# Lingeng56/conformer-pytorch-lightning

Hardware: AMD Instinct MI355X
Metric: encoder frames/sec (80-d fbank, T=1000), whole job (higher is better)
Workload: dtype bf16

## Files before the change

conformer-pytorch-lightning_amd/cfm/__init__.py:

```python
import ctypes
import os
import threading

import torch

_HERE = os.path.dirname(os.path.abspath(__file__))
LIB_PATH = os.path.join(os.path.dirname(_HERE), "libconformer_gfx950.so")

F32, BF16, F16 = 0, 1, 2
ACT_NONE, ACT_SILU, ACT_RELU, ACT_GLU, ACT_DSILU, ACT_DRELU = 0, 1, 2, 3, 4, 5
TILE_AUTO_TRAIN = -1

_DT = {torch.float32: F32, torch.bfloat16: BF16, torch.float16: F16}
_TORCH_DT = {F32: torch.float32, BF16: torch.bfloat16, F16: torch.float16}

c_p = ctypes.c_void_p
c_i64 = ctypes.c_int64
c_i32 = ctypes.c_int32
c_f = ctypes.c_float


class GemmDesc(ctypes.Structure):
    _fields_ = [("A", c_p), ("W", c_p), ("W_lo", c_p), ("bias", c_p), ("residual", c_p), ("row_mask", c_p), ("C", c_p),
                ("lda", c_i64), ("ldc", c_i64), ("ldr", c_i64),
# ... 134 lines not shown
    _fields_ = [("lat", Lattice), ("logits", c_p), ("ld", c_i64), ("logits_dtype", c_i32), ("V", c_i32), ("blank", c_i32), ("ld_targets", c_i32),
                ("targets", c_p), ("lse", c_p), ("lp_blank", c_p), ("lp_label", c_p), ("alpha", c_p), ("beta", c_p), ("shift", c_p),
                ("nll", c_p), ("nll_shifted", c_p), ("ll_alpha", c_p),
                ("grad", c_p), ("ld_grad", c_i64), ("grad_dtype", c_i32), ("grad_cols", c_i32), ("gscale", ctypes.c_float),
                ("gscale_stride", c_i32), ("gscale_dev", c_p), ("clamp", ctypes.c_float)]


class LnBwdDesc(ctypes.Structure):
    _fields_ = [("x", c_p), ("dy", c_p), ("gamma", c_p), ("row_mask", c_p), ("dres", c_p), ("dx", c_p), ("dgamma", c_p), ("dbeta", c_p), ("ws", c_p),
                ("dx2", c_p), ("M", c_i64), ("D", c_i32), ("dy_dtype", c_i32), ("dx2_dtype", c_i32), ("accumulate", c_i32),
                ("eps", ctypes.c_float), ("alpha2", ctypes.c_float), ("p1", ctypes.c_float), ("p2", ctypes.c_float),
                ("seed1", ctypes.c_uint32), ("seed2", ctypes.c_uint32), ("dx2_row_mask", c_p),
                ("chain_x", c_p), ("chain_gamma", c_p), ("chain_dgamma", c_p), ("chain_dbeta", c_p)]


class GreedyDesc(ctypes.Structure):
    _fields_ = [("embed", c_p), ("lstm_w", c_p * 4), ("lstm_b", c_p * 4), ("proj_w", c_p), ("proj_b", c_p), ("pf_w", c_p), ("pf_b", c_p), ("out_w", c_p),
                ("out_b", c_p), ("enc_proj", c_p), ("token", c_p), ("t", c_p), ("count", c_p), ("frame_count", c_p), ("hyps", c_p), ("lens", c_p),
                ("h", c_p), ("c", c_p), ("h_new", c_p), ("c_new", c_p), ("pred", c_p), ("act", c_p), ("pmax", c_p), ("pidx", c_p), ("done", c_p),
                ("n_done", c_p), ("hyp_cap", c_i64), ("hyp_ld", c_i64), ("B", c_i32), ("T", c_i32), ("L", c_i32), ("E", c_i32), ("H", c_i32),
                ("P", c_i32), ("J", c_i32), ("Vp", c_i32), ("blank", c_i32), ("n_steps", c_i32)]


class GreedyChunkDesc(ctypes.Structure):
    _fields_ = ([("embed", c_p), ("lstm_w", c_p * 4), ("lstm_b", c_p * 4)] +
                [(n, c_p) for n in ("proj_w", "proj_b", "pf_w", "pf_b", "out_w", "out_b", "ef_w", "ef_b", "enc", "enc_proj", "token", "t", "count", "frame_count",
                                    "hyps", "lens", "h", "c", "h_new", "c_new", "pred", "pp", "act", "pmax", "pidx", "rows", "row_off", "row_cnt", "n_rows",
                                    "steps", "overflow", "done", "n_done")] +
                [("hyp_cap", c_i64), ("hyp_ld", c_i64)] +
                [(n, c_i32) for n in ("B", "chunk", "L", "E", "H", "P", "J", "D", "Vp", "blank", "n_steps", "carry")])


class FbankDesc(ctypes.Structure):
    _fields_ = ([(n, c_p) for n in ("samples", "lengths", "feats_length", "carry_in", "carry_out", "fresh_in", "pos_in", "fresh_out", "pos_out", "twiddle", "window",
                                    "mel_w", "mel_start", "mel_len", "mel_off", "out")] + [("ld", c_i64)] +
                [(n, c_i32) for n in ("B", "n_cols", "rows", "F", "win", "shift", "padded", "mel_nnz", "samples_i16", "carry_n", "hop")] +
                [("dither", c_f), ("seed", ctypes.c_uint32)])


class FfnSplitDesc(ctypes.Structure):
    _fields_ = [("x", c_p), ("psum", c_p), ("psum_b2", c_p), ("psum_splits", c_i32), ("psum_alpha", c_f), ("ln1_g", c_p), ("ln1_b", c_p), ("ln2_g", c_p),
                ("ln2_b", c_p), ("rows_out", c_p), ("rows2_out", c_p), ("ln_g", c_p), ("ln_b", c_p), ("w1", c_p), ("b1", c_p), ("N1", c_i32), ("act", c_i32),
                ("w2", c_p), ("psum_out", c_p), ("out16", c_p), ("ldo", c_i64), ("M", c_i32), ("D", c_i32), ("mode", c_i32), ("w_dtype", c_i32), ("eps", c_f),
                ("kv_ring", c_p), ("ring_offsets", c_p), ("ring_T", c_i32), ("ring_H", c_i32), ("ring_Tq", c_i32)]


class LayerScratch(ctypes.Structure):
    _fields_ = [(n, c_p) for n in ("xn", "hid", "qkv", "pos", "ctx", "glu", "dw")] + [("psum", c_p), ("psum_splits", c_i32)]


class LayerIO(ctypes.Structure):
    _fields_ = [("B", c_i32), ("T", c_i32), ("D", c_i32), ("H", c_i32), ("FF", c_i32), ("ktaps", c_i32),
                ("act_dtype", c_i32), ("w_dtype", c_i32),
                ("attn_mask", c_p), ("am_sb", c_i64), ("am_sq", c_i64),
                ("pad_valid", c_p), ("pos_embed", c_p), ("pos_rows", c_i32),
                ("pos_proj", c_p), ("pos_proj_ld", c_i64),
                ("attn_cache", c_p), ("cache_T", c_i32), ("new_cache", c_p), ("after_g", c_p), ("after_b", c_p), ("after_out", c_p),
                ("kv_ring", c_p), ("stream_offset", c_p), ("ring_T", c_i32), ("causal_conv", c_i32), ("conv_cache", c_p), ("pos_shared", c_i32),
                ("next_w", c_p), ("next_x_out", c_p), ("macaron_done", c_i32)]


ROUTES = ("GENERAL", "FUSED_FFN", "CHAIN", "CHAIN_NEXT", "CHAIN_NEXT_CIN", "FFSPLIT", "PAIR")

_lib = None
_lock = threading.Lock()


def lib():
    global _lib
    if _lib is not None:
        return _lib
    with _lock:
        if _lib is not None:
            return _lib
        if not os.path.exists(LIB_PATH):
            raise RuntimeError(
                "libconformer_gfx950.so not found at %s -- build it with `python -c 'import __graft_entry__ as g; g.build()'` "
                "or `make -C conformer-pytorch-lightning_amd/csrc`. There is no CPU fallback." % LIB_PATH)
        L = ctypes.CDLL(LIB_PATH)
        L.cfm_version.restype = ctypes.c_int
        L.cfm_last_error.restype = ctypes.c_char_p
        L.cfm_device_ok.restype = ctypes.c_int
        L.cfm_gemm.argtypes = [ctypes.POINTER(GemmDesc), c_p]
        L.cfm_attention.argtypes = [ctypes.POINTER(AttnDesc), c_p]
        L.cfm_ffn_fused.argtypes = [ctypes.POINTER(FfnDesc), c_p]
        L.cfm_rowchain.argtypes = [ctypes.POINTER(RowChainDesc), c_p]
        L.cfm_rowchain_supported.argtypes = [c_i32, c_i32]
        L.cfm_rowchain_pair_supported.argtypes = [c_i32, c_i32]
        L.cfm_layernorm.argtypes = [c_p, c_p, c_p, c_p, c_i32, c_p, c_p, c_p, c_i32, c_p, ctypes.c_float, c_i64, c_i32, c_p]
        L.cfm_kv_cache_pack.argtypes = [c_p, c_i32, c_p, c_p, c_i32, c_i64, c_i64, c_i64, c_i64, c_p, c_i32, c_i32, c_i32, c_i32, c_p]
        L.cfm_dwconv_bn_silu.argtypes = [c_p, c_i32, c_p, c_p, c_p, c_p, c_p, c_i32, c_i32, c_i32, c_i32, c_i32, c_p]
        L.cfm_conv1_relu.argtypes = [c_p, c_p, c_p, c_p, c_i32, c_i32, c_i32, c_i32, c_i32, c_p, c_p, c_p]
        L.cfm_conv1_relu_mma.argtypes = [c_p, c_p, c_p, c_p, c_i32, c_i32, c_i32, c_i32, c_i32, c_p, c_p, c_p]
        L.cfm_conv12_supported.argtypes = [c_i32, c_i32]
        L.cfm_pack_matrices.argtypes = [c_p, c_i32, c_i64, c_i32, c_i32, c_p]
        L.cfm_pack_vectors.argtypes = [c_p, c_p, c_p, c_i64, c_p]
        L.cfm_greedy_step.argtypes = [ctypes.POINTER(GreedyDesc), c_p]
        L.cfm_greedy_chunk_begin.argtypes = [ctypes.POINTER(GreedyChunkDesc), c_p]
        L.cfm_greedy_chunk_step.argtypes = [ctypes.POINTER(GreedyChunkDesc), c_p]
        L.cfm_fbank.argtypes = [ctypes.POINTER(FbankDesc), c_p]
        L.cfm_fbank_stream.argtypes = [ctypes.POINTER(FbankDesc), c_p]
        L.cfm_ffn_split.argtypes = [ctypes.POINTER(FfnSplitDesc), c_p]
        L.cfm_ffn_split_supported.argtypes = [c_i32, c_i32]
        L.cfm_attention_bwd_force_general.argtypes = [c_i32]
        L.cfm_attention_bwd_force_general.restype = None
        L.cfm_set_cin_merge.argtypes = [c_i32]
        L.cfm_set_cin_merge.restype = c_i32
        L.cfm_set_conv12_tile.argtypes = [c_i32]
        L.cfm_set_conv12_tile.restype = c_i32
        L.cfm_conv12_plan.argtypes = [c_i64, c_i32, c_i32, ctypes.POINTER(c_i32), ctypes.POINTER(c_i32)]
        L.cfm_dwconv_bn_train_bwd_acc.argtypes = [c_p, c_i32, c_p, c_p, c_p, c_i32, c_p, c_p, c_i32, c_p, c_p, c_p, c_p, c_p, c_p, c_i32, c_i32, c_i32, c_i32, c_i32, c_p]
        L.cfm_layernorm_bwd_fused.argtypes = [ctypes.POINTER(LnBwdDesc), c_p]
        L.cfm_conv12_relu.argtypes = [c_p, c_p, c_p, c_p, c_p, c_p, c_i32, c_i32, c_i32, c_i32, c_i32, c_p, c_p, c_p]
        L.cfm_valid_mask.argtypes = [c_p, c_i32, c_p, c_i32, c_i32, c_i32, c_i32, c_p]
        L.cfm_chunk_mask.argtypes = [c_p, c_i32, c_i32, c_i32, c_p]
        L.cfm_attn_mask.argtypes = [c_p, c_p, c_p, c_i32, c_i32, c_p]
        L.cfm_cast.argtypes = [c_p, c_i32, c_p, c_i32, c_i64, c_p]
        L.cfm_add_rows.argtypes = [c_p, c_p, c_i64, c_i32, c_i32, c_p]
        L.cfm_encoder_layer_forward.argtypes = [ctypes.POINTER(LayerWeights), ctypes.POINTER(LayerScratch),
                                                ctypes.POINTER(LayerIO), c_p, c_p, c_i32, c_p, c_p, c_p]
        L.cfm_encoder_layer_route.argtypes = [ctypes.POINTER(LayerWeights), ctypes.POINTER(LayerScratch), ctypes.POINTER(LayerIO), c_p, c_p]
        L.cfm_encoder_layer_route.restype = c_i32
        L.cfm_ffsplit_max_rows.restype = c_i32
        L.cfm_ctc_nll.argtypes = [c_p, c_i64, c_i32, c_i32, c_i32, c_p, c_p, c_i32, c_p, c_p, c_p, c_p]
        L.cfm_joint_act.argtypes = [c_p, c_i64, c_p, c_i64, c_p, c_i32, c_i32, c_i32, c_i32, c_i32, c_p]
        L.cfm_joint_act_bwd.argtypes = [c_p, c_i64, c_p, c_i64, c_p, c_p, c_p, c_p, c_i32, c_i32, c_i32, c_i32, c_p]
        L.cfm_joint_act_bwd_ws.argtypes = [c_i32, c_i32, c_i32, c_i32]
        L.cfm_rnnt_nll.argtypes = [ctypes.POINTER(RnntDesc), c_p]
        L.cfm_rnnt_grad.argtypes = [ctypes.POINTER(RnntDesc), c_p]
        L.cfm_rnnt_packed_nll.argtypes = [ctypes.POINTER(RnntPackedDesc), c_p]
        L.cfm_rnnt_packed_grad.argtypes = [ctypes.POINTER(RnntPackedDesc), c_p]
        L.cfm_joint_act_packed.argtypes = [c_p, c_i64, c_p, c_i64, c_p, c_i32, ctypes.POINTER(Lattice), c_i32, c_p]
        L.cfm_joint_act_packed_bwd.argtypes = [c_p, c_i64, c_p, c_i64, c_p, c_p, c_p, c_p, ctypes.POINTER(Lattice), c_i32, c_p]
        c_f = ctypes.c_float
        L.cfm_gemm_tn.argtypes = [ctypes.POINTER(GemmTnDesc), c_p]
        L.cfm_gemm_tn_group.argtypes = [ctypes.POINTER(GemmTnDesc), c_i32, c_p]
        L.cfm_attention_bwd.argtypes = [ctypes.POINTER(AttnBwdDesc), c_p]
        L.cfm_layernorm_bwd_ws.argtypes = [c_i64, c_i32]
        L.cfm_layernorm_bwd.argtypes = [c_p, c_p, c_i32, c_p, c_p, c_p, c_p, c_p, c_p, c_p, c_f, c_i64, c_i32, c_p]
        L.cfm_glu_bwd.argtypes = [c_p, c_i32, c_p, c_i32, c_p, c_i32, c_i64, c_i32, c_p]
        L.cfm_dwconv_bn_ws.argtypes = [c_i32, c_i32, c_i32]
        L.cfm_dwconv_bn_train.argtypes = [c_p, c_i32, c_p, c_p, c_p, c_p, c_p, c_p, c_f, c_f, c_p, c_p, c_p, c_i32, c_p, c_i32, c_i32, c_i32, c_i32, c_p]
        L.cfm_dwconv_bn_train_bwd.argtypes = [c_p, c_i32, c_p, c_p, c_p, c_i32, c_p, c_p, c_i32, c_p, c_p, c_p, c_p, c_p, c_p, c_i32, c_i32, c_i32, c_i32, c_p]
        L.cfm_col2im_relu_bwd.argtypes = [c_p, c_i32, c_p, c_i32, c_p, c_i32, c_i32, c_i32, c_i32, c_i32, c_p]
        L.cfm_conv1_wgrad_ws.argtypes = [c_i32, c_i32, c_i32]
        L.cfm_conv1_wgrad.argtypes = [c_p, c_i32, c_p, c_p, c_p, c_p, c_p, c_p, c_i32, c_i32, c_i32, c_i32, c_p]
        L.cfm_ctc_nll_train_groups.argtypes = [ctypes.POINTER(CtcGroup), c_i32, c_i32, c_p]
        L.cfm_ctc_grad.argtypes = [c_p, c_i64, c_i32, c_i32, c_i32, c_p, c_p, c_i32, c_p, c_p, c_p, c_p, c_p, c_p, c_f, c_p, c_p, c_p]
        L.cfm_adam_step.argtypes = [c_p, c_p, c_p, c_p, c_i64, c_f, c_f, c_f, c_f, c_f, c_i64, c_p, c_p]
        L.cfm_sumsq.argtypes = [c_p, c_i64, c_p, c_i32, c_p, c_p]
        L.cfm_adam_clip_step.argtypes = [c_p, c_p, c_p, c_p, c_i64, c_f, c_f, c_f, c_f, c_f, c_i64, c_p, c_f, c_f, c_i32, c_p, c_p]
        L.cfm_dropout_rows.argtypes = [c_p, c_i32, c_p, c_i32, c_p, c_f, c_f, ctypes.c_uint32, c_f, ctypes.c_uint32, c_i64, c_i32, c_p]
        L.cfm_dropout_mask.argtypes = [c_p, c_i64, c_f, ctypes.c_uint32, c_p]
        L.cfm_encoder_train_forward.argtypes = [c_i32, ctypes.POINTER(LayerTrainWeights), ctypes.POINTER(LayerTrainIO), ctypes.POINTER(LayerTrainSaved),
                                                ctypes.POINTER(LayerTrainScratch), ctypes.POINTER(c_p), c_p]
        L.cfm_encoder_train_backward.argtypes = [c_i32, ctypes.POINTER(LayerTrainWeights), ctypes.POINTER(LayerTrainIO), ctypes.POINTER(LayerTrainSaved),
                                                 ctypes.POINTER(LayerTrainScratch), ctypes.POINTER(LayerTrainGrads), ctypes.POINTER(c_p), c_p, c_p, c_p,
                                                 LAYER_DONE_FN, c_p, ctypes.POINTER(c_p), c_p]
        L.cfm_stream_prep.argtypes = [c_p, c_i32, c_i32, c_i32, c_i32, c_p, c_i32, c_i32, c_p, c_p, c_p, c_p]
        L.cfm_kv_ring_write.argtypes = [c_p, c_p, c_i32, c_i64, c_i64, c_i64, c_i64, c_p, c_p, c_i32, c_i32, c_i32, c_i32, c_i32, c_p]
        L.cfm_stream_advance.argtypes = [c_p, c_p, c_i32, c_i32, c_p]
        L.cfm_dwconv_causal_bn_silu.argtypes = [c_p, c_i32, c_p, c_p, c_p, c_p, c_p, c_p, c_i32, c_i32, c_i32, c_i32, c_i32, c_p]
        L.cfm_conv_cache_update.argtypes = [c_p, c_i32, c_p, c_i32, c_i32, c_i32, c_i32, c_p]
        for name in ("cfm_layernorm_bwd_ws", "cfm_dwconv_bn_ws", "cfm_conv1_wgrad_ws", "cfm_joint_act_bwd_ws"):
            getattr(L, name).restype = c_i64
        L.cfm_prof_enable.argtypes = [c_i32]
        L.cfm_prof_enable.restype = None
        L.cfm_prof_reset.restype = None
        L.cfm_prof_collect.restype = ctypes.c_int
        L.cfm_prof_entry.argtypes = [c_i32, ctypes.c_char_p, c_i32, ctypes.POINTER(c_i64), ctypes.POINTER(ctypes.c_double),
                                     ctypes.POINTER(ctypes.c_double), ctypes.POINTER(ctypes.c_double)]
        for name in ("cfm_gemm", "cfm_ffn_fused", "cfm_rowchain", "cfm_rowchain_supported", "cfm_attention", "cfm_layernorm", "cfm_kv_cache_pack", "cfm_dwconv_bn_silu", "cfm_conv1_relu", "cfm_conv1_relu_mma", "cfm_conv12_relu", "cfm_conv12_supported",
                     "cfm_valid_mask", "cfm_chunk_mask", "cfm_attn_mask", "cfm_cast", "cfm_add_rows",
                     "cfm_encoder_layer_forward", "cfm_ctc_nll", "cfm_joint_act", "cfm_joint_act_bwd", "cfm_rnnt_nll", "cfm_rnnt_grad", "cfm_prof_entry", "cfm_gemm_tn", "cfm_gemm_tn_group", "cfm_attention_bwd",
                     "cfm_layernorm_bwd", "cfm_glu_bwd", "cfm_dwconv_bn_train", "cfm_dwconv_bn_train_bwd", "cfm_col2im_relu_bwd", "cfm_conv1_wgrad",
                     "cfm_ctc_nll_train_groups", "cfm_ctc_grad", "cfm_adam_step", "cfm_adam_clip_step", "cfm_sumsq", "cfm_dropout_rows", "cfm_dropout_mask", "cfm_pack_matrices", "cfm_pack_vectors", "cfm_greedy_step", "cfm_greedy_chunk_begin", "cfm_greedy_chunk_step", "cfm_fbank", "cfm_fbank_stream", "cfm_ffn_split", "cfm_ffn_split_supported", "cfm_layernorm_bwd_fused", "cfm_dwconv_bn_train_bwd_acc",
                     "cfm_encoder_train_forward", "cfm_encoder_train_backward", "cfm_stream_prep", "cfm_kv_ring_write", "cfm_stream_advance", "cfm_dwconv_causal_bn_silu", "cfm_conv_cache_update"):
            getattr(L, name).restype = ctypes.c_int
        _lib = L
    return _lib


def check(rc, what):
    if rc != 0:
        raise RuntimeError("%s failed (status %d): %s" % (what, rc, lib().cfm_last_error().decode(errors="replace")))


def dt_code(t):
    try:
        return _DT[t.dtype if isinstance(t, torch.Tensor) else t]
    except KeyError:
        raise TypeError("cfm: unsupported dtype %s (float32, bfloat16, float16 only)" % (t.dtype if isinstance(t, torch.Tensor) else t))


def torch_dtype(code):
    return _TORCH_DT[code]


def require_hip(*tensors):
    for t in tensors:
        if t is None:
            continue
        if not t.is_cuda:
            raise RuntimeError("cfm: tensor on %s -- this framework runs on MI355X (HIP) only; there is no CPU path" % t.device)


def ptr(t):
    return None if t is None else t.data_ptr()


def stream():
    return torch.cuda.current_stream().cuda_stream


class Precision:

    def __init__(self, name):
        if name not in ("bf16", "fp16", "fp32"):
            raise ValueError("precision must be bf16, fp16 or fp32, got %r" % (name,))
        self.name = name
        self.split = name == "fp32"
        self.w_code = F16 if name == "fp16" else BF16
        self.act_code = F32 if self.split else self.w_code
        self.w_dtype = torch_dtype(self.w_code)
        self.act_dtype = torch_dtype(self.act_code)

    def __repr__(self):
        return "Precision(%s)" % self.name


_precision = Precision(os.environ.get("CFM_PRECISION", "bf16"))


def set_precision(name):
    global _precision
    _precision = name if isinstance(name, Precision) else Precision(name)
    return _precision


def get_precision():
    return _precision


def resolve_precision(module=None):
    p = getattr(module, "precision", None) if module is not None else None
    if p is None:
        return _precision
    return p if isinstance(p, Precision) else Precision(p)


_warned = set()


def check_mode(module, what):
    if module.training:
# ... 11 lines not shown
```

conformer-pytorch-lightning_amd/cfm/ops.py:

```python
import ctypes

import torch

import cfm as _c

__all__ = ["fbank", "fbank_stream", "stream_prep", "stream_advance", "dwconv_causal_bn_silu", "conv_cache_update", "dropout_rows", "dropout_mask", "set_deterministic", "gemm_tn", "gemm_tn_group", "layernorm_bwd", "glu_bwd", "dwconv_bn_train", "dwconv_bn_train_bwd", "col2im_relu_bwd", "conv1_wgrad", "attention_bwd",
           "ctc_nll_train_groups", "ctc_grad", "rnnt_nll", "rnnt_grad", "joint_act_bwd", "rnnt_nll_packed", "joint_act_packed", "joint_act_packed_bwd", "ffn_split", "adam_step", "adam_clip_step", "sumsq", "scratch_stats",
           "gemm", "ffn_fused", "ffn_fused_supported", "rowchain", "rowchain_supported", "rowchain_pair_supported", "layernorm", "attention", "kv_cache_pack", "dwconv_bn_silu", "conv1_relu", "conv1_relu_mma_supported", "conv12_relu", "conv12_supported", "ctc_nll", "joint_act", "valid_mask", "chunk_mask",
           "attn_mask_combine", "cast", "add_rows", "scratch", "prof_enable", "prof_reset", "prof_table", "as_u8_mask"]


def _rows2d(t, name):
    if t.dim() != 2 or t.stride(1) != 1:
        raise ValueError("cfm.%s: expected a 2-D tensor with unit inner stride, got shape %s strides %s" % (name, tuple(t.shape), t.stride()))
    return t


_arena = {}
_retired = []


def scratch(tag, numel, dtype, device):
    device = torch.device(device)
    key = (tag, dtype, device, torch.cuda.current_stream(device).cuda_stream)
    buf = _arena.get(key)
    if buf is None or buf.numel() < numel:
        want = max(int(numel), 1) if buf is None else max(int(numel), buf.numel() * 3 // 2)
        if buf is not None:
            _retired.append(buf)
        buf = torch.empty(want, dtype=dtype, device=device)
        _arena[key] = buf
    return buf[:numel]


def scratch_stats():
    held = sum(b.numel() * b.element_size() for b in list(_arena.values()) + _retired)
    return len(_arena), len(_retired), held


def gemm(a, w, bias=None, w_lo=None, out=None, out_dtype=None, act=_c.ACT_NONE, residual=None, alpha=1.0, row_mask=None,
         mask_mode=0, conv=None, tile=0, n_out=None, pre_out=None, aux=None, drop=None, drop2=None):
    _c.require_hip(a, w, bias, w_lo, out, residual, row_mask)
    w = _rows2d(w, "gemm(w)")
    N, K = w.shape
    d = _c.GemmDesc()
    if conv is None:
        a = _rows2d(a, "gemm(a)")
        M = a.shape[0]
        if a.shape[1] != K:
            raise ValueError("cfm.gemm: a is %s but w is %s" % (tuple(a.shape), tuple(w.shape)))
        d.lda = a.stride(0)
    else:
        C, T1, F1, T2, F2, M = conv
        if not a.is_contiguous():
            raise ValueError("cfm.gemm(conv): image must be contiguous channels-last [B,T1,F1,C]")
        d.conv_C, d.conv_T1, d.conv_F1, d.conv_T2, d.conv_F2 = C, T1, F1, T2, F2
        d.lda = 0
    cols = N // 2 if act == _c.ACT_GLU else N
    if out is None:
        odt = out_dtype if out_dtype is not None else (residual.dtype if residual is not None else torch.float32)
        out = torch.empty((M, cols), dtype=odt, device=a.device)
    else:
        out = _rows2d(out, "gemm(out)")
        if out.shape[0] != M or out.shape[1] != cols:
            raise ValueError("cfm.gemm: out is %s, expected (%d,%d)" % (tuple(out.shape), M, cols))
    if residual is not None:
        residual = _rows2d(residual, "gemm(residual)")
        if residual.dtype != torch.float32 or out.dtype != torch.float32 or tuple(residual.shape) != (M, cols):
            raise ValueError("cfm.gemm: residual accumulate needs f32 residual/out of shape (%d,%d)" % (M, cols))
        d.ldr = residual.stride(0)
    if bias is not None and (bias.dtype != torch.float32 or bias.numel() != N or not bias.is_contiguous()):
        raise ValueError("cfm.gemm: bias must be contiguous f32 [N]")
    if row_mask is not None and (row_mask.dtype != torch.uint8 or row_mask.numel() != M or not row_mask.is_contiguous()):
        raise ValueError("cfm.gemm: row_mask must be contiguous uint8 [M]")
    if w_lo is not None and (w_lo.shape != w.shape or w_lo.dtype != w.dtype or not w_lo.is_contiguous()):
        raise ValueError("cfm.gemm: w_lo must match w")
    if pre_out is not None:
        _c.require_hip(pre_out)
        pre_out = _rows2d(pre_out, "gemm(pre_out)")
        if tuple(pre_out.shape) != (M, N):
            raise ValueError("cfm.gemm: pre_out is %s, expected (%d,%d)" % (tuple(pre_out.shape), M, N))
        d.C_pre, d.ld_pre, d.pre_dtype = _c.ptr(pre_out), pre_out.stride(0), _c.dt_code(pre_out)
    if aux is not None:
        _c.require_hip(aux)
        aux = _rows2d(aux, "gemm(aux)")
        if tuple(aux.shape) != (M, N):
            raise ValueError("cfm.gemm: aux is %s, expected (%d,%d)" % (tuple(aux.shape), M, N))
        d.aux, d.ld_aux, d.aux_dtype = _c.ptr(aux), aux.stride(0), _c.dt_code(aux)
    if drop is not None and drop[0] > 0.0:
        d.drop_p, d.drop_seed = float(drop[0]), int(drop[1]) & 0xFFFFFFFF
        if drop2 is not None and drop2[0] > 0.0:
            d.drop2_p, d.drop2_seed = float(drop2[0]), int(drop2[1]) & 0xFFFFFFFF
    d.A, d.W, d.W_lo, d.bias, d.residual, d.row_mask, d.C = _c.ptr(a), _c.ptr(w), _c.ptr(w_lo), _c.ptr(bias), _c.ptr(residual), _c.ptr(row_mask), _c.ptr(out)
    d.ldc = out.stride(0)
    d.M, d.N, d.K = M, N, K
    d.a_dtype, d.w_dtype, d.c_dtype = _c.dt_code(a), _c.dt_code(w), _c.dt_code(out)
    d.act, d.alpha, d.tile, d.mask_mode = act, alpha, tile, mask_mode
    _c.check(_c.lib().cfm_gemm(ctypes.byref(d), _c.stream()), "cfm_gemm")
    return out


def ffn_fused_supported(D, FF, prec):
    return (not prec.split) and D in (144, 256) and FF % 32 == 0 and FF <= 2048


def ffn_fused(x, w1f, w2f, b1, b2, FF, act=_c.ACT_SILU, ln=None, alpha=1.0, add_x=False, ln1=None, ln2=None, out_f32=None,
              want_f32=True, out16_dtype=None, eps=1e-5):
    _c.require_hip(x, w1f, w2f, b1, b2, out_f32)
    x = _rows2d(x, "ffn_fused(x)")
    if x.dtype != torch.float32 or not x.is_contiguous():
        raise ValueError("cfm.ffn_fused: x must be contiguous float32 [M,D]")
    M, D = x.shape
    d = _c.FfnDesc()
    d.x, d.w1f, d.w2f, d.b1, d.b2 = _c.ptr(x), _c.ptr(w1f), _c.ptr(w2f), _c.ptr(b1), _c.ptr(b2)
    for name, pair in (("ln", ln), ("ln1", ln1), ("ln2", ln2)):
        if pair is not None:
            setattr(d, name + "_g", _c.ptr(pair[0]))
            setattr(d, name + "_b", _c.ptr(pair[1]))
    if want_f32 and out_f32 is None:
        out_f32 = torch.empty((M, D), dtype=torch.float32, device=x.device)
    out16 = torch.empty((M, D), dtype=out16_dtype, device=x.device) if out16_dtype is not None else None
    d.out_f32, d.out16 = _c.ptr(out_f32), _c.ptr(out16)
    d.M, d.D, d.FF = M, D, FF
    d.w_dtype = _c.dt_code(w1f)
    d.out16_dtype = _c.dt_code(out16) if out16 is not None else 0
    d.act, d.add_x, d.alpha, d.eps = act, 1 if add_x else 0, alpha, eps
    _c.check(_c.lib().cfm_ffn_fused(ctypes.byref(d), _c.stream()), "cfm_ffn_fused")
    return out_f32, out16


def rowchain_supported(D, FF, prec):
    return (not prec.split) and bool(_c.lib().cfm_rowchain_supported(D, FF))


def rowchain_pair_supported(D, FF, prec):
    return (not prec.split) and bool(_c.lib().cfm_rowchain_pair_supported(D, FF))


def ffn_split(x, w_code, mode, psum=None, psum_b2=None, psum_alpha=1.0, ln1=None, ln2=None, rows_out=None, rows2_out=None, ln=None, w1=None, b1=None,
              n1=0, act=_c.ACT_NONE, w2=None, psum_out=None, out16=None, eps=1e-5, ring=None):
    _c.require_hip(x, psum, psum_b2, rows_out, rows2_out, w1, b1, w2, psum_out, out16)
    x = _rows2d(x, "ffn_split(x)")
    M, D = x.shape
    if x.dtype != torch.float32 or not x.is_contiguous():
        raise ValueError("cfm.ffn_split: x must be contiguous float32 rows")
    d = _c.FfnSplitDesc()
    d.x, d.M, d.D, d.mode, d.w_dtype, d.eps = x.data_ptr(), M, D, mode, w_code, eps
    if psum is not None:
        if psum.dtype != torch.float32 or psum.dim() != 3 or tuple(psum.shape[1:]) != (M, D) or not psum.is_contiguous():
            raise ValueError("cfm.ffn_split: psum must be contiguous float32 [G, M, D]")
        d.psum, d.psum_b2, d.psum_splits, d.psum_alpha = psum.data_ptr(), _c.ptr(psum_b2), psum.shape[0], psum_alpha
    for name, pair in (("ln1", ln1), ("ln2", ln2), ("ln", ln)):
        if pair is not None:
            setattr(d, name + "_g", pair[0].data_ptr())
            setattr(d, name + "_b", pair[1].data_ptr())
    d.rows_out, d.rows2_out = _c.ptr(rows_out), _c.ptr(rows2_out)
    d.w1, d.b1, d.N1, d.act, d.w2, d.psum_out = _c.ptr(w1), _c.ptr(b1), n1, act, _c.ptr(w2), _c.ptr(psum_out)
    if out16 is not None:
        d.out16, d.ldo = out16.data_ptr(), out16.stride(0)
    if ring is not None:
        kv, offs, tq = ring
        _c.require_hip(kv, offs)
        d.kv_ring, d.ring_offsets, d.ring_T, d.ring_H, d.ring_Tq = kv.data_ptr(), offs.data_ptr(), kv.shape[2], kv.shape[1], tq
    _c.check(_c.lib().cfm_ffn_split(ctypes.byref(d), _c.stream()), "cfm_ffn_split")


def rowchain(M, D, w_code, x=None, head=None, ln=None, ln_mask=None, ffn=None, alpha=1.0, ln1=None, ln2=None, out_f32=None, out16=None,
             tail=None, eps=1e-5, dw=None):
    d = _c.RowChainDesc()
    keep = [x, out_f32, out16, ln_mask]
    d.x, d.out_f32, d.out16, d.ln_mask = _c.ptr(x), _c.ptr(out_f32), _c.ptr(out16), _c.ptr(ln_mask)
    if head is not None:
        a16, hw, hb, res, hm = head
        _c.require_hip(a16, hw, hb, res, hm)
        d.head_a, d.head_w, d.head_b, d.head_res, d.head_mask = _c.ptr(a16), _c.ptr(hw), _c.ptr(hb), _c.ptr(res), _c.ptr(hm)
        keep += list(head)
    for name, pair in (("ln", ln), ("ln1", ln1), ("ln2", ln2)):
        if pair is not None:
            setattr(d, name + "_g", _c.ptr(pair[0]))
            setattr(d, name + "_b", _c.ptr(pair[1]))
    if ffn is not None:
        d.w1f, d.w2n, d.b1, d.b2, d.FF = _c.ptr(ffn[0]), _c.ptr(ffn[1]), _c.ptr(ffn[2]), _c.ptr(ffn[3]), ffn[4]
    if tail is not None:
        d.tail_w, d.tail_b, d.tail_N, d.tail_glu, d.tail_out = _c.ptr(tail[0]), _c.ptr(tail[1]), tail[2], 1 if tail[3] else 0, _c.ptr(tail[4])
# ... 727 lines not shown
```

conformer-pytorch-lightning_amd/convolution.py:

```python
import torch
import torch.nn as nn

import cfm
from cfm import packing

_NO_CACHE = torch.zeros((0, 0, 0, 0))


def _rows_f32(t):
    t = t.reshape(-1, t.size(-1))
    return (t if t.dtype == torch.float32 else t.float()).contiguous()


class ConvolutionModule(nn.Module):

    def __init__(self, input_dim, kernel_size, bias=True):
        super().__init__()
        bias = bool(bias)
        self.pointwise_conv1 = nn.Conv1d(input_dim, 2 * input_dim, kernel_size=1, stride=1, padding=0, bias=bias)
        self.glu = nn.GLU(dim=1)
        self.depthwise_conv = nn.Conv1d(input_dim, input_dim, kernel_size=kernel_size, stride=1,
                                        padding=(kernel_size - 1) // 2, groups=input_dim, bias=bias)
        self.norm = nn.BatchNorm1d(input_dim)
        self.activation = nn.SiLU()
        self.pointwise_conv2 = nn.Conv1d(input_dim, input_dim, kernel_size=1, stride=1, padding=0)
        self._pack = packing.PackCache()
        self.causal = False

    def forward(self, inputs, inputs_pad_mask, cache=_NO_CACHE):
        cfm.require_hip(inputs)
        prec = cfm.resolve_precision(self)
        B, T, D = inputs.shape
        keep = None
        if inputs_pad_mask is not None and inputs_pad_mask.dim() >= 3 and inputs_pad_mask.size(2) > 0:
            keep = cfm.as_u8_mask(inputs_pad_mask).reshape(-1)
            if keep.numel() != B * T:
                raise RuntimeError("pad mask %s does not match inputs %s" % (tuple(inputs_pad_mask.shape), tuple(inputs.shape)))
        if cfm.check_mode(self, "ConvolutionModule"):
            from cfm import autograd as ag
            out = ag.ConvModuleFn.apply(inputs, self, prec, keep, *self.parameters())
            return out, torch.zeros((0, 0, 0), dtype=inputs.dtype, device=inputs.device)
        pk = packing.pack_conv_module(self, prec)
        x = _rows_f32(inputs)
        glu = cfm.gemm(x, pk.pw1_w, bias=pk.pw1_b, w_lo=pk.pw1_w_lo, act=cfm.ACT_GLU, row_mask=keep, mask_mode=1,
                       out_dtype=prec.act_dtype)
        if self.causal:
            K = self.depthwise_conv.kernel_size[0]
            have = cache is not None and cache.dim() == 3 and cache.size(0) > 0
            ctx = cache.to(device=inputs.device, dtype=torch.float32).contiguous() if have else None
            dw = cfm.dwconv_causal_bn_silu(glu.view(B, T, D), pk.dw_w, pk.dw_b, pk.bn_scale, pk.bn_shift, cache=ctx)
            new_ctx = ctx.clone() if have else torch.zeros((B, K - 1, D), dtype=torch.float32, device=inputs.device)
            cfm.conv_cache_update(glu.view(B, T, D), new_ctx, K)
            out = cfm.gemm(dw.view(B * T, D), pk.pw2_w, bias=pk.pw2_b, w_lo=pk.pw2_w_lo, row_mask=keep, mask_mode=0, out_dtype=torch.float32)
            return out.view(B, T, D).to(inputs.dtype), new_ctx
        dw = cfm.dwconv_bn_silu(glu.view(B, T, D), pk.dw_w, pk.dw_b, pk.bn_scale, pk.bn_shift)
        out = cfm.gemm(dw.view(B * T, D), pk.pw2_w, bias=pk.pw2_b, w_lo=pk.pw2_w_lo, row_mask=keep, mask_mode=0,
                       out_dtype=torch.float32)
        new_cache = torch.zeros((0, 0, 0), dtype=inputs.dtype, device=inputs.device)
        return out.view(B, T, D).to(inputs.dtype), new_cache


FUSE_CONVS = True


class ConvolutionSubSampling(nn.Module):

    def __init__(self, input_dim, output_dim, pos_enc):
        super().__init__()
        self.conv = nn.Sequential(
            nn.Conv2d(1, output_dim, 3, 2),
            nn.ReLU(),
            nn.Conv2d(output_dim, output_dim, 3, 2),
            nn.ReLU(),
        )
        self.out = nn.Sequential(nn.Linear(output_dim * (((input_dim - 1) // 2 - 1) // 2), output_dim))
        self.pos_enc = pos_enc
        self._pack = packing.PackCache()

    def embed_frames(self, inputs, cmvn=None):
        cfm.require_hip(inputs)
        prec = cfm.resolve_precision(self)
        if cfm.check_mode(self, "ConvolutionSubSampling"):
            from cfm import autograd as ag
            return ag.SubsamplingFn.apply(inputs, self, prec, cmvn, *ag.subsampling_params(self))
        pk = packing.pack_subsampling(self, prec)
        x = (inputs if inputs.dtype == torch.float32 else inputs.float()).contiguous()
        B, T, F = x.shape
        C = pk.C
        T1, F1 = (T - 3) // 2 + 1, (F - 3) // 2 + 1
        T2, F2 = (T1 - 3) // 2 + 1, (F1 - 3) // 2 + 1
        if T2 < 1 or F2 != pk.Fp:
            raise RuntimeError("input of shape %s is too short / has the wrong feature size for this front-end" % (tuple(inputs.shape),))
        if FUSE_CONVS and pk.w2_lo is None and cfm.conv12_supported(C, prec.act_dtype):
            h2 = cfm.conv12_relu(x, pk.w1, pk.b1, pk.w2, pk.b2, cmvn=cmvn)
        else:
            h1 = cfm.conv1_relu(x, pk.w1, pk.b1, prec.act_dtype, cmvn=cmvn,
                                mma=cfm.conv1_relu_mma_supported(C, prec.act_dtype))
            h2 = cfm.gemm(h1, pk.w2, bias=pk.b2, w_lo=pk.w2_lo, act=cfm.ACT_RELU, conv=(C, T1, F1, T2, F2, B * T2 * F2),
                          out_dtype=prec.act_dtype)
        y = cfm.gemm(h2.view(B * T2, F2 * C), pk.wl, bias=pk.bl, w_lo=pk.wl_lo, out_dtype=torch.float32)
        return y.view(B, T2, -1)

    def forward(self, inputs, inputs_pad_mask, offset=0):
        y = self.embed_frames(inputs).to(inputs.dtype)
        y, pos_embed = self.pos_enc(y, offset)
        return y, pos_embed, inputs_pad_mask[:, :, 2::2][:, :, 2::2]

    def position_encoding(self, offset, size):
        return self.pos_enc.position_encoding(offset, size)
```

include/cfm.h:

```cpp
#ifndef CFM_H_
#define CFM_H_

#include <stddef.h>
#include <stdint.h>

#ifdef __cplusplus
extern "C" {
#endif

#define CFM_VERSION 306

typedef void* cfm_stream_t;

typedef enum { CFM_F32 = 0, CFM_BF16 = 1, CFM_F16 = 2 } cfm_dtype;

typedef enum {
    CFM_OK = 0,
    CFM_ERR_ARG = -1,
    CFM_ERR_LAUNCH = -2,
    CFM_ERR_UNSUPPORTED = -3
} cfm_status;

typedef enum {
    CFM_ACT_NONE = 0, CFM_ACT_SILU = 1, CFM_ACT_RELU = 2, CFM_ACT_GLU = 3,
    CFM_ACT_DSILU = 4, CFM_ACT_DRELU = 5
} cfm_act;

int cfm_version(void);
const char* cfm_last_error(void);
int cfm_device_ok(void);

#define CFM_TILE_AUTO_TRAIN (-1)
typedef struct {
    const void* A;
    const void* W;
    const void* W_lo;
    const float* bias;
    const float* residual;
    const uint8_t* row_mask;
    void* C;
    int64_t lda, ldc, ldr;
    int32_t M, N, K;
    int32_t a_dtype, w_dtype, c_dtype;
    int32_t act;
    float alpha;
    int32_t conv_C, conv_T1, conv_F1, conv_T2, conv_F2;
    int32_t tile;
    int32_t mask_mode;
    void* C_pre;
    int64_t ld_pre;
    int32_t pre_dtype;
    int32_t aux_dtype;
    const void* aux;
    int64_t ld_aux;
    float drop_p, drop2_p;
    uint32_t drop_seed, drop2_seed;
} cfm_gemm_desc;

int cfm_gemm(const cfm_gemm_desc* d, cfm_stream_t stream);

typedef struct {
    const void* A;
    const void* B;
    float* C;
    float* colsum;
    const uint8_t* row_mask;
    int64_t lda, ldb, ldc;
    int32_t M, N, K;
    int32_t a_dtype, b_dtype, mma_dtype;
    int32_t split, accumulate, splits;
    float alpha;
    int32_t conv_C, conv_T1, conv_F1, conv_T2, conv_F2;
    const int64_t* row_off;
    const int64_t* colsum_off;
    int32_t tile;
    const int64_t* colsum_off2;
} cfm_gemm_tn_desc;

int cfm_gemm_tn(const cfm_gemm_tn_desc* d, cfm_stream_t stream);
int cfm_gemm_tn_group(const cfm_gemm_tn_desc* descs, int32_t n, cfm_stream_t stream);

typedef struct {
    const float* x;
    const float *ln_g, *ln_b;
    const void *w1f, *w2f;
    const float *b1, *b2;
    const float *ln1_g, *ln1_b, *ln2_g, *ln2_b;
    float* out_f32;
    void* out16;
    int64_t M;
    int32_t D, FF;
    int32_t w_dtype, out16_dtype;
    int32_t act;
    int32_t add_x;
    float alpha, eps;
} cfm_ffn_desc;

int cfm_ffn_fused(const cfm_ffn_desc* d, cfm_stream_t stream);

typedef struct {
    const float* x;
    const void* head_a;
    const void* head_w;
    const float* head_b;
    const float* head_res;
    const uint8_t* head_mask;
    const float *ln_g, *ln_b;
    const uint8_t* ln_mask;
    const void *w1f, *w2n;
    const float *b1, *b2;
    const float *ln1_g, *ln1_b, *ln2_g, *ln2_b;
    float* out_f32;
    void* out16;
    const void* tail_w;
    const float* tail_b;
    void* tail_out;
    int64_t M;
    int32_t D, FF, tail_N, tail_glu;
    int32_t w_dtype;
    float alpha, eps;
    float* out2_f32;
    const float *dw_w, *dw_b, *dw_scale, *dw_shift;
    int32_t dw_T, dw_K;
    const float *s2_ln_g, *s2_ln_b;
    const void *s2_w1f, *s2_w2n;
    const float *s2_b1, *s2_b2;
    float* s2_out_f32;
    float s2_alpha;
    float* psum_out;
    const float* psum_in;
    const float* psum_b2;
    float psum_alpha;
    const void *cin_a, *cin_w;
    const float *cin_b, *cin_res;
    float* cin_out;
    const float *cin_ln_g, *cin_ln_b;
    const uint8_t* cin_mask;
    const void* cin_tail_w;
    const float* cin_tail_b;
    int32_t tail_pair;
} cfm_rowchain_desc;

// ... 456 lines not shown
```

Before: 27.17 million.

## Add dedicated pipelined GEMM kernel for subsampling front-end linear projection

```diff
diff --git a/conformer-pytorch-lightning_amd/cfm/__init__.py b/conformer-pytorch-lightning_amd/cfm/__init__.py
--- a/conformer-pytorch-lightning_amd/cfm/__init__.py
+++ b/conformer-pytorch-lightning_amd/cfm/__init__.py
@@ -240,6 +240,8 @@
         L.cfm_last_error.restype = ctypes.c_char_p
         L.cfm_device_ok.restype = ctypes.c_int
         L.cfm_gemm.argtypes = [ctypes.POINTER(GemmDesc), c_p]
+        L.cfm_front_linear.argtypes = [c_p, c_i64, c_p, c_p, c_p, c_i64, c_i32, c_i32, c_i32, c_i32, c_p]
+        L.cfm_front_linear_supported.argtypes = [c_i32, c_i32, c_i32, c_i32]
         L.cfm_attention.argtypes = [ctypes.POINTER(AttnDesc), c_p]
         L.cfm_ffn_fused.argtypes = [ctypes.POINTER(FfnDesc), c_p]
         L.cfm_rowchain.argtypes = [ctypes.POINTER(RowChainDesc), c_p]
@@ -328,7 +330,7 @@
         L.cfm_prof_collect.restype = ctypes.c_int
         L.cfm_prof_entry.argtypes = [c_i32, ctypes.c_char_p, c_i32, ctypes.POINTER(c_i64), ctypes.POINTER(ctypes.c_double),
                                      ctypes.POINTER(ctypes.c_double), ctypes.POINTER(ctypes.c_double)]
-        for name in ("cfm_gemm", "cfm_ffn_fused", "cfm_rowchain", "cfm_rowchain_supported", "cfm_attention", "cfm_layernorm", "cfm_kv_cache_pack", "cfm_dwconv_bn_silu", "cfm_conv1_relu", "cfm_conv1_relu_mma", "cfm_conv12_relu", "cfm_conv12_supported",
+        for name in ("cfm_gemm", "cfm_front_linear", "cfm_front_linear_supported", "cfm_ffn_fused", "cfm_rowchain", "cfm_rowchain_supported", "cfm_attention", "cfm_layernorm", "cfm_kv_cache_pack", "cfm_dwconv_bn_silu", "cfm_conv1_relu", "cfm_conv1_relu_mma", "cfm_conv12_relu", "cfm_conv12_supported",
                      "cfm_valid_mask", "cfm_chunk_mask", "cfm_attn_mask", "cfm_cast", "cfm_add_rows",
                      "cfm_encoder_layer_forward", "cfm_ctc_nll", "cfm_joint_act", "cfm_joint_act_bwd", "cfm_rnnt_nll", "cfm_rnnt_grad", "cfm_prof_entry", "cfm_gemm_tn", "cfm_gemm_tn_group", "cfm_attention_bwd",
                      "cfm_layernorm_bwd", "cfm_glu_bwd", "cfm_dwconv_bn_train", "cfm_dwconv_bn_train_bwd", "cfm_col2im_relu_bwd", "cfm_conv1_wgrad",
diff --git a/conformer-pytorch-lightning_amd/cfm/ops.py b/conformer-pytorch-lightning_amd/cfm/ops.py
--- a/conformer-pytorch-lightning_amd/cfm/ops.py
+++ b/conformer-pytorch-lightning_amd/cfm/ops.py
@@ -6,7 +6,7 @@
 
 __all__ = ["fbank", "fbank_stream", "stream_prep", "stream_advance", "dwconv_causal_bn_silu", "conv_cache_update", "dropout_rows", "dropout_mask", "set_deterministic", "gemm_tn", "gemm_tn_group", "layernorm_bwd", "glu_bwd", "dwconv_bn_train", "dwconv_bn_train_bwd", "col2im_relu_bwd", "conv1_wgrad", "attention_bwd",
            "ctc_nll_train_groups", "ctc_grad", "rnnt_nll", "rnnt_grad", "joint_act_bwd", "rnnt_nll_packed", "joint_act_packed", "joint_act_packed_bwd", "ffn_split", "adam_step", "adam_clip_step", "sumsq", "scratch_stats",
-           "gemm", "ffn_fused", "ffn_fused_supported", "rowchain", "rowchain_supported", "rowchain_pair_supported", "layernorm", "attention", "kv_cache_pack", "dwconv_bn_silu", "conv1_relu", "conv1_relu_mma_supported", "conv12_relu", "conv12_supported", "ctc_nll", "joint_act", "valid_mask", "chunk_mask",
+           "gemm", "front_linear", "front_linear_supported", "ffn_fused", "ffn_fused_supported", "rowchain", "rowchain_supported", "rowchain_pair_supported", "layernorm", "attention", "kv_cache_pack", "dwconv_bn_silu", "conv1_relu", "conv1_relu_mma_supported", "conv12_relu", "conv12_supported", "ctc_nll", "joint_act", "valid_mask", "chunk_mask",
            "attn_mask_combine", "cast", "add_rows", "scratch", "prof_enable", "prof_reset", "prof_table", "as_u8_mask"]
 
 
@@ -100,6 +100,24 @@
     return out
 
 
+def front_linear_supported(M, N, K, dtype, w_lo=None):
+    return w_lo is None and dtype in (torch.bfloat16, torch.float16) and bool(_c.lib().cfm_front_linear_supported(M, N, K, _c.dt_code(dtype)))
+
+
+def front_linear(a, w, bias=None):
+    _c.require_hip(a, w, bias)
+    a, w = _rows2d(a, "front_linear(a)"), _rows2d(w, "front_linear(w)")
+    M, (N, K) = a.shape[0], w.shape
+    if a.shape[1] != K or a.dtype != w.dtype or not w.is_contiguous():
+        raise ValueError("cfm.front_linear: a is %s %s but w is %s %s" % (tuple(a.shape), a.dtype, tuple(w.shape), w.dtype))
+    if bias is not None and (bias.dtype != torch.float32 or bias.numel() != N or not bias.is_contiguous()):
+        raise ValueError("cfm.front_linear: bias must be contiguous f32 [N]")
+    out = torch.empty((M, N), dtype=torch.float32, device=a.device)
+    _c.check(_c.lib().cfm_front_linear(_c.ptr(a), a.stride(0), _c.ptr(w), _c.ptr(bias), _c.ptr(out), out.stride(0), M, N, K, _c.dt_code(a), _c.stream()),
+             "cfm_front_linear")
+    return out
+
+
 def ffn_fused_supported(D, FF, prec):
     return (not prec.split) and D in (144, 256) and FF % 32 == 0 and FF <= 2048
 
diff --git a/conformer-pytorch-lightning_amd/convolution.py b/conformer-pytorch-lightning_amd/convolution.py
--- a/conformer-pytorch-lightning_amd/convolution.py
+++ b/conformer-pytorch-lightning_amd/convolution.py
@@ -98,7 +98,11 @@
                                 mma=cfm.conv1_relu_mma_supported(C, prec.act_dtype))
             h2 = cfm.gemm(h1, pk.w2, bias=pk.b2, w_lo=pk.w2_lo, act=cfm.ACT_RELU, conv=(C, T1, F1, T2, F2, B * T2 * F2),
                           out_dtype=prec.act_dtype)
-        y = cfm.gemm(h2.view(B * T2, F2 * C), pk.wl, bias=pk.bl, w_lo=pk.wl_lo, out_dtype=torch.float32)
+        rows = h2.view(B * T2, F2 * C)
+        if cfm.front_linear_supported(B * T2, pk.wl.shape[0], F2 * C, h2.dtype, w_lo=pk.wl_lo):
+            y = cfm.front_linear(rows, pk.wl, bias=pk.bl)
+        else:
+            y = cfm.gemm(rows, pk.wl, bias=pk.bl, w_lo=pk.wl_lo, out_dtype=torch.float32)
         return y.view(B, T2, -1)
 
     def forward(self, inputs, inputs_pad_mask, offset=0):
diff --git a/conformer-pytorch-lightning_amd/csrc/frontlinear.hip b/conformer-pytorch-lightning_amd/csrc/frontlinear.hip
--- /dev/null
+++ b/conformer-pytorch-lightning_amd/csrc/frontlinear.hip
@@ -0,0 +1,182 @@
+#include <string>
+#include <type_traits>
+
+#include "cfm_common.h"
+
+namespace {
+
+#define CFM_INL __attribute__((always_inline))
+
+struct FrontLinearArgs {
+    const u16* A;
+    const u16* W;
+    const float* bias;
+    float* C;
+    int64_t lda, ldc;
+    int M, N, K;
+};
+
+template <int N>
+__device__ __forceinline__ void wait_vm() {
+    __builtin_amdgcn_s_waitcnt((N & 15) | (7 << 4) | (15 << 8) | ((N >> 4) << 14));
+    asm volatile("" ::: "memory");
+}
+__device__ __forceinline__ void wait_lgkm0() {
+    __builtin_amdgcn_s_waitcnt(15 | (7 << 4) | (0 << 8) | (3 << 14));
+}
+
+template <typename HT, int BM, int BN, int WM, int WN, int NS>
+__global__ __launch_bounds__(64 * WM * WN) void cfm_front_linear_kernel(const FrontLinearArgs g) {
+    constexpr int BK = 64, NW = WM * WN;
+    constexpr int A_CH = BM * 8, W_CH = BN * 8;
+    constexpr int STAGE = A_CH + W_CH;
+    constexpr int FM = BM / WM / 16, FN = BN / WN / 16;
+    constexpr int A_BLK = BM / 8, W_BLK = BN / 8;
+    constexpr int LPT = (A_BLK + W_BLK) / NW;
+    static_assert(A_BLK % NW == 0 && W_BLK % NW == 0, "a request is either an activation or a weight block for every wavefront");
+    static_assert(NS >= 3 && LPT * (NS - 2) < 64, "ring depth: the counted waits fit vmcnt");
+    static_assert(STAGE * NS * 16 <= 160 * 1024, "the ring fits the LDS");
+    __shared__ u32x4 smem[NS * STAGE];
+
+    const int tid = threadIdx.x, lane = tid & 63;
+    const int wave = __builtin_amdgcn_readfirstlane(tid >> 6);
+    const int wr = wave / WN, wc = wave % WN;
+    const int tiles_n = g.N / BN, tiles_m = (g.M + BM - 1) / BM;
+    const int per_group = 8 * tiles_n;
+    const int grp = blockIdx.x / per_group, rem = blockIdx.x - grp * per_group;
+    const int tile_m = grp * 8 + (rem & 7);
+    if (tile_m >= tiles_m) return;
+    const int m0 = tile_m * BM, n0 = (rem >> 3) * BN;
+
+    unsigned src_off[LPT];
+#pragma unroll
+    for (int i = 0; i < LPT; ++i) {
+        const int q = i * NW + wave;
+        const bool is_a = i * NW < A_BLK;
+        const int r = (is_a ? q : q - A_BLK) * 8 + (lane >> 3);
+        const int c = (lane & 7) ^ ((r >> 1) & 7);
+        if (is_a) {
+            int m = m0 + r;
+            m = m < g.M ? m : g.M - 1;
+            src_off[i] = ((unsigned)((int64_t)m * g.lda) + c * 8) * 2u;
+        } else {
+            src_off[i] = ((unsigned)(n0 + r) * (unsigned)g.K + c * 8) * 2u;
+        }
+    }
+    auto stage = [&](int buf, int kt) CFM_INL {
+        const unsigned kb = (unsigned)(kt * BK) * 2u;
+        u32x4* const dst = smem + buf * STAGE;
+#pragma unroll
+        for (int i = 0; i < LPT; ++i) {
+            const char* base = i * NW < A_BLK ? (const char*)g.A : (const char*)g.W;
+            __builtin_amdgcn_global_load_lds((const __attribute__((address_space(1))) void*)(base + (src_off[i] + kb)),
+                                             (__attribute__((address_space(3))) void*)(dst + (i * NW + wave) * 64), 16, 0, 0);
+        }
+    };
+
+    const int q4 = (lane >> 4) * 4;
+    f32x4 bias_r[FN];
+#pragma unroll
+    for (int j = 0; j < FN; ++j) {
+        const int col = n0 + wc * (BN / WN) + j * 16 + q4;
+        bias_r[j] = g.bias ? *(const f32x4*)(g.bias + col) : (f32x4){0.f, 0.f, 0.f, 0.f};
+    }
+
+    f32x4 acc[FM][FN];
+#pragma unroll
+    for (int i = 0; i < FM; ++i)
+#pragma unroll
+        for (int j = 0; j < FN; ++j) acc[i][j] = (f32x4){0.f, 0.f, 0.f, 0.f};
+    const int sw = (lane >> 1) & 7;
+    const int a_row = wr * (BM / WM) + (lane & 15), w_row = wc * (BN / WN) + (lane & 15);
+    auto read_frags = [&](int buf, int kk, u32x4 (&af)[FM], u32x4 (&wf)[FN]) CFM_INL {
+        const u32x4* const As = smem + buf * STAGE;
+        const u32x4* const Ws = As + A_CH;
+        const int c = (kk * 4 + (lane >> 4)) ^ sw;
+#pragma unroll
+        for (int j = 0; j < FN; ++j) wf[j] = Ws[(w_row + j * 16) * 8 + c];
+#pragma unroll
+        for (int i = 0; i < FM; ++i) af[i] = As[(a_row + i * 16) * 8 + c];
+    };
+    auto mma = [&](const u32x4 (&af)[FM], const u32x4 (&wf)[FN]) CFM_INL {
+        __builtin_amdgcn_s_setprio(1);
+#pragma unroll
+        for (int i = 0; i < FM; ++i)
+#pragma unroll
+            for (int j = 0; j < FN; ++j) acc[i][j] = HT::mfma(wf[j], af[i], acc[i][j]);
+        __builtin_amdgcn_s_setprio(0);
+    };
+
+    const int nkt = g.K / BK;
+#pragma unroll
+    for (int t = 0; t < NS - 1; ++t)
+        if (t < nkt) stage(t, t);
+    if (nkt >= NS - 1) wait_vm<LPT * (NS - 2)>();
+    else wait_vm<0>();
+    __builtin_amdgcn_s_barrier();
+    __builtin_amdgcn_sched_barrier(0);
+    u32x4 af0[FM], wf0[FN], af1[FM], wf1[FN];
+    read_frags(0, 0, af0, wf0);
+    int rd = 0, wrb = NS - 1;
+    for (int kt = 0; kt < nkt; ++kt) {
+        const bool more = kt + NS - 1 < nkt;
+        wait_lgkm0();
+        if (more) wait_vm<LPT * (NS - 3)>();
+        else wait_vm<0>();
+        __builtin_amdgcn_s_barrier();
+        __builtin_amdgcn_sched_barrier(0);
+        if (more) stage(wrb, kt + NS - 1);
+        read_frags(rd, 1, af1, wf1);
+        mma(af0, wf0);
+        const int rn = rd + 1 == NS ? 0 : rd + 1;
+        read_frags(rn, 0, af0, wf0);
+        mma(af1, wf1);
+        rd = rn;
+        wrb = wrb + 1 == NS ? 0 : wrb + 1;
+    }
+
+    const int col0 = n0 + wc * (BN / WN) + q4;
+#pragma unroll
+    for (int i = 0; i < FM; ++i) {
+        const int row = m0 + wr * (BM / WM) + i * 16 + (lane & 15);
+        if (row >= g.M) continue;
+        float* const rowp = g.C + (int64_t)row * g.ldc + col0;
+#pragma unroll
+        for (int j = 0; j < FN; ++j) {
+            f32x4 v = acc[i][j];
+            v += bias_r[j];
+            *(f32x4*)(rowp + j * 16) = v;
+        }
+    }
+}
+
+template <typename HT, int BM, int BN, int WM, int WN, int NS>
+int launch(const FrontLinearArgs& a, hipStream_t s, const char* name) {
+    const int grid = (((a.M + BM - 1) / BM + 7) / 8) * 8 * (a.N / BN);
+    const double flops = 2.0 * a.M * (double)a.N * a.K;
+    const double bytes = (double)a.M * a.K * 2 + (double)a.N * a.K * 2 + (double)a.M * a.N * 4;
+    CfmProfScope prof(name, s, flops, bytes);
+    CFM_LAUNCH((cfm_front_linear_kernel<HT, BM, BN, WM, WN, NS>), dim3(grid), dim3(64 * WM * WN), 0, s, a);
+    return cfm_launch_status(name);
+}
+
+}
+
+extern "C" int cfm_front_linear_supported(int32_t M, int32_t N, int32_t K, int32_t dtype) {
+    return M > 0 && N == 256 && K >= 64 && K % 64 == 0 && (dtype == CFM_BF16 || dtype == CFM_F16);
+}
+
+extern "C" int cfm_front_linear(const void* A, int64_t lda, const void* W, const float* bias, float* C, int64_t ldc, int32_t M, int32_t N,
+                                int32_t K, int32_t dtype, cfm_stream_t stream) {
+    CFM_CHECK_ARG(A && W && C, "cfm_front_linear: null pointer");
+    CFM_CHECK_ARG(cfm_front_linear_supported(M, N, K, dtype), "cfm_front_linear: needs 16-bit operands, N == 256 and K %% 64 == 0 (M=%d N=%d K=%d dtype=%d)",
+                  M, N, K, dtype);
+    CFM_CHECK_ARG(lda >= K && lda % 8 == 0 && ldc >= N && ldc % 4 == 0, "cfm_front_linear: lda=%lld must be a multiple of 8, ldc=%lld of 4",
+                  (long long)lda, (long long)ldc);
+    CFM_CHECK_ARG(((int64_t)(M - 1) * lda + K) * 2 < ((int64_t)1 << 32) && (int64_t)N * K * 2 < ((int64_t)1 << 32),
+                  "cfm_front_linear: operand too large for 32-bit byte offsets");
+    FrontLinearArgs a;
+    a.A = (const u16*)A; a.W = (const u16*)W; a.bias = bias; a.C = C; a.lda = lda; a.ldc = ldc; a.M = M; a.N = N; a.K = K;
+    hipStream_t s = (hipStream_t)stream;
+    return dtype == CFM_BF16 ? launch<BF16, 64, 128, 2, 4, 5>(a, s, "gemm_front_bf16") : launch<F16, 64, 128, 2, 4, 5>(a, s, "gemm_front_f16");
+}
diff --git a/include/cfm.h b/include/cfm.h
--- a/include/cfm.h
+++ b/include/cfm.h
@@ -58,6 +58,10 @@
 } cfm_gemm_desc;
 
 int cfm_gemm(const cfm_gemm_desc* d, cfm_stream_t stream);
+
+int cfm_front_linear_supported(int32_t M, int32_t N, int32_t K, int32_t dtype);
+int cfm_front_linear(const void* A, int64_t lda, const void* W, const float* bias, float* C, int64_t ldc, int32_t M, int32_t N, int32_t K,
+                     int32_t dtype, cfm_stream_t stream);
 
 typedef struct {
     const void* A;
```

New measurement: 27.25 million (median of 4 runs). No clear change (+0.3%).
